# eriksandstroem/Loopy-SLAM

Hardware: AMD Instinct MI355X
Metric: rays/s (track+map, Replica room0 per-frame budget, 640x480 synthetic RGB-D) (higher is better)
Workload: dtype f32 (decoder products as split products on the 16-bit matrix pipe: fp16x3 forward, bf16x6 / pre-scaled fp16x3 backward, fp32 accumulate; weight gradients on pre-scaled fp16x3 too)

## Files before the change

### loopy_slam_amd/csrc/lk_bwd2.hip

```cpp
#include "lk_common.h"
#include "lk_kernels.h"
#include "lk_adam_dev.h"
#include "lk_exposure_dev.h"

using namespace lkw;

LK_CHAIN_DEFINE(bwd2)

__device__ __forceinline__ void interp_bwd_block(const LkInterpBwdArgs& a, int block) {
    const int sub = (int)threadIdx.x & 7;
    const int p_raw = block * 32 + ((int)threadIdx.x >> 3);
    const bool live = p_raw < a.P;
    const int pidx = live ? p_raw : a.P - 1;
    const bool has = a.nbr_count[pidx] >= a.min_nn;
    const bool color = (a.flags & LK_FLAG_STAGE_COLOR) != 0;
    const bool relpos = (a.flags & LK_FLAG_REL_POS) != 0;
    const bool do_col = color && !relpos;
    int id[LK_K];
    float w[LK_K];
    {
        const int4 i0 = *reinterpret_cast<const int4*>(a.nbr_idx + (size_t)pidx * LK_K);
        const int4 i1 = *reinterpret_cast<const int4*>(a.nbr_idx + (size_t)pidx * LK_K + 4);
        const float4 w0 = *reinterpret_cast<const float4*>(a.nbr_w + (size_t)pidx * LK_K);
        const float4 w1 = *reinterpret_cast<const float4*>(a.nbr_w + (size_t)pidx * LK_K + 4);
        id[0] = i0.x; id[1] = i0.y; id[2] = i0.z; id[3] = i0.w; id[4] = i1.x; id[5] = i1.y; id[6] = i1.z; id[7] = i1.w;
        w[0] = w0.x; w[1] = w0.y; w[2] = w0.z; w[3] = w0.w; w[4] = w1.x; w[5] = w1.y; w[6] = w1.z; w[7] = w1.w;
    }
    const float4 dcg = *reinterpret_cast<const float4*>(a.dc_geo + (size_t)pidx * LK_C + sub * 4);
    float4 dcc = make_float4(0.f, 0.f, 0.f, 0.f);
    if (do_col) dcc = *reinterpret_cast<const float4*>(a.dc_col + (size_t)pidx * LK_C + sub * 4);
    if (!(a.flags & LK_FLAG_GRAD_RAYS)) return;
    float dwn[LK_K];
#pragma unroll
    for (int j = 0; j < LK_K; ++j) {
        float part = 0.0f;
        if (has && w[j] != 0.0f) {
            const float4 g = lk_feat4(a.geo_feats, (a.flags & LK_FLAG_FEATS_F16) != 0, (size_t)id[j] * LK_C + sub * 4);
            part = dcg.x * g.x + dcg.y * g.y + dcg.z * g.z + dcg.w * g.w;
            if (do_col) {
                const float4 c = lk_feat4(a.col_feats, (a.flags & LK_FLAG_FEATS_F16) != 0, (size_t)id[j] * LK_C + sub * 4);
                part += dcc.x * c.x + dcc.y * c.y + dcc.z * c.z + dcc.w * c.w;
            }
        }
        part = lk_sum8<true>(part);
        if (color && relpos && a.dw_rel && has) part += a.dw_rel[(size_t)pidx * LK_K + j];
        dwn[j] = part;
    }
    LK_STAMPW(7);
    const int r = pidx / a.S;
    const float z = a.z[pidx];
    const float px = lk_madd_rn(a.rays_o[3 * r], a.rays_d[3 * r], z);
    const float py = lk_madd_rn(a.rays_o[3 * r + 1], a.rays_d[3 * r + 1], z);
    const float pz = lk_madd_rn(a.rays_o[3 * r + 2], a.rays_d[3 * r + 2], z);
    const float r2 = a.r2_ray ? a.r2_ray[r] : a.r2_static;
    float dpx = 0.0f, dpy = 0.0f, dpz = 0.0f;
    if (has) {
        float wr[LK_K], ex[LK_K], ey[LK_K], ez[LK_K];
        float S = 0.0f, dot = 0.0f;
#pragma unroll
        for (int j = 0; j < LK_K; ++j) {
            wr[j] = 0.0f; ex[j] = ey[j] = ez[j] = 0.0f;
            if (id[j] >= 0) {
                const float x = a.pos[3 * (size_t)id[j]], y = a.pos[3 * (size_t)id[j] + 1], zz = a.pos[3 * (size_t)id[j] + 2];
                const float D = lk_dist2(px, py, pz, x, y, zz);
                if (D <= r2) { wr[j] = 1.0f / (D + 1e-10f); ex[j] = x - px; ey[j] = y - py; ez[j] = zz - pz; }
            }
            S += wr[j];
            dot += dwn[j] * w[j];
        }
        const float invS = 1.0f / fmaxf(S, 1e-12f);
#pragma unroll
        for (int j = 0; j < LK_K; ++j) {
            if (wr[j] != 0.0f) {
                const float dw = (dwn[j] - dot) * invS;
                const float dD = -wr[j] * wr[j] * dw;
                dpx += dD * (-2.0f) * ex[j]; dpy += dD * (-2.0f) * ey[j]; dpz += dD * (-2.0f) * ez[j];
            }
        }
    }
    if (live && sub == 0) {
        if (a.dp_embed) { const float4 e = *reinterpret_cast<const float4*>(a.dp_embed + (size_t)pidx * 4); dpx += e.x; dpy += e.y; dpz += e.z; }
        if (color && a.dp_embed_col) { const float4 e = *reinterpret_cast<const float4*>(a.dp_embed_col + (size_t)pidx * 4); dpx += e.x; dpy += e.y; dpz += e.z; }
        if (color && relpos && a.dp_rel) { const float4 e = *reinterpret_cast<const float4*>(a.dp_rel + (size_t)pidx * 4); dpx += e.x; dpy += e.y; dpz += e.z; }
        *reinterpret_cast<float4*>(a.dp_total + (size_t)pidx * 4) = make_float4(dpx, dpy, dpz, 0.0f);
    }
    LK_STAMPW(8);
    if (a.pose_part) {
        __shared__ float s_pp[4][12];
        float v[12];
        const bool mine = live && sub == 0;
        const float d0 = mine ? (a.pix_i[r] - a.cx) / a.fx : 0.0f, d1 = mine ? -(a.pix_j[r] - a.cy) / a.fy : 0.0f, d2 = mine ? -1.0f : 0.0f;
        const float gx = mine ? dpx : 0.0f, gy = mine ? dpy : 0.0f, gz = mine ? dpz : 0.0f;
        const float zx = gx * z, zy = gy * z, zz = gz * z;
        v[0] = zx * d0; v[1] = zx * d1; v[2] = zx * d2; v[3] = zy * d0; v[4] = zy * d1; v[5] = zy * d2; v[6] = zz * d0; v[7] = zz * d1; v[8] = zz * d2;
        v[9] = gx; v[10] = gy; v[11] = gz;
#pragma unroll
        for (int q = 0; q < 12; ++q) {
#pragma unroll
            for (int o = 32; o >= 8; o >>= 1) v[q] += __shfl_xor(v[q], o);
        }
        const int wv = (int)threadIdx.x >> 6;
        if (lk_lane() == 0) {
#pragma unroll
            for (int q = 0; q < 12; ++q) s_pp[wv][q] = v[q];
        }
        __syncthreads();
        if (threadIdx.x < 12) a.pose_part[(size_t)block * 12 + threadIdx.x] = (s_pp[0][threadIdx.x] + s_pp[1][threadIdx.x]) + (s_pp[2][threadIdx.x] + s_pp[3][threadIdx.x]);
    }
    LK_STAMPW(9);
}
__global__ __launch_bounds__(256) void k_interp_bwd(LkInterpBwdArgs a) { interp_bwd_block(a, (int)blockIdx.x); }
__global__ __launch_bounds__(256) void k_interp_bwd_x(LkInterpBwdArgs a, ExposureStepArgs xa, const float* __restrict__ part, int n_part) {
    if (blockIdx.x + 1 == gridDim.x) { lk_exposure_step_body(xa, part, n_part); return; }
    interp_bwd_block(a, (int)blockIdx.x);
}

__global__ __launch_bounds__(256) void k_seg_count(LkFeatScatterArgs a) {
    const long long row = (long long)blockIdx.x * 256 + (int)threadIdx.x;
    if (row >= (long long)a.P * LK_K) return;
    const int y = (int)blockIdx.y;
    const long long grow = (long long)y * a.P * LK_K + row;
    const int s = (int)(row >> 3);
    const int idx = a.nbr_idx[grow];
    int rk = -1;
    const bool skipped = a.live_rays && s >= a.live_rays[y] * a.S;
    if (!skipped && idx >= 0 && a.nbr_w[grow] != 0.0f && a.nbr_count[(size_t)y * a.P + s] >= a.min_nn && (!a.row_mask || a.row_mask[idx])) {
        const int key = a.key_of ? a.key_of[idx] : idx;
        if (key >= 0) rk = atomicAdd(a.seg_cnt + (size_t)y * a.cnt_stride + key, 1);
    }
    a.seg_rank[grow] = rk;
}
__global__ __launch_bounds__(256) void k_seg_place(LkFeatScatterArgs a) {
    const long long row = (long long)blockIdx.x * 256 + (int)threadIdx.x;
    if (row >= (long long)a.P * LK_K) return;
    const int y = (int)blockIdx.y;
    const long long base = (long long)y * a.P * LK_K;
    const int32_t* __restrict__ off = a.seg_off + (size_t)y * a.cnt_stride;
    const int rk = a.seg_rank[base + row];
    if (rk >= 0) {
        const int idx = a.nbr_idx[base + row];
        a.seg_list[base + off[a.key_of ? a.key_of[idx] : idx] + rk] = (int)row;
    }
    if (row == 0 && a.seg_total) a.seg_total[y] = off[a.N];
}

__global__ __launch_bounds__(256) void k_seg_rank_det(LkFeatScatterArgs a) {
    const long long row = (long long)blockIdx.x * 256 + (int)threadIdx.x;
    if (row >= (long long)a.P * LK_K) return;
    const int y = (int)blockIdx.y;
    const long long base = (long long)y * a.P * LK_K;
    if (a.seg_rank[base + row] < 0) return;
    const int32_t* __restrict__ off = a.seg_off + (size_t)y * a.cnt_stride;
    const int idx = a.nbr_idx[base + row];
    const int key = a.key_of ? a.key_of[idx] : idx;
    int rk = 0;
    for (int i = off[key], e = off[key + 1]; i < e; ++i) rk += a.seg_list[base + i] < (int)row;
    a.seg_rank[base + row] = rk;
}

#define LK_DW2_LDS_SAMPLES 32
__device__ __forceinline__ void dw2_body(const float* __restrict__ dc, const float* __restrict__ w_sum, const float* __restrict__ hbar,
                                         int P_all, const int32_t* __restrict__ live_rays, int S, float* __restrict__ part, int bx, int nb) {
    const int P = live_rays ? min(P_all, *live_rays * S) : P_all;
    __shared__ __attribute__((aligned(16))) float s_h[LK_DW2_LDS_SAMPLES][128];
    __shared__ float s_a[LK_DW2_LDS_SAMPLES][33];
    const int t = (int)threadIdx.x, n = t >> 3, k0 = 16 * (t & 7);
    float acc[16], bsum = 0.0f;
#pragma unroll
    for (int i = 0; i < 16; ++i) acc[i] = 0.0f;
    for (int s0 = bx * 64; s0 < P; s0 += nb * 64) {
        for (int half = 0; half < 64; half += LK_DW2_LDS_SAMPLES) {
            const int ns = min(LK_DW2_LDS_SAMPLES, P - s0 - half);
            if (ns <= 0) break;
            __syncthreads();
#pragma unroll
            for (int q = 0; q < LK_DW2_LDS_SAMPLES * 32 / 256; ++q) {
                const int e = q * 256 + t, sm = e >> 5;
                float4 v = make_float4(0.f, 0.f, 0.f, 0.f);
                float av = 0.0f;
                if (sm < ns) {
                    v = reinterpret_cast<const float4*>(hbar + (size_t)(s0 + half + sm) * 128)[e & 31];
                    av = w_sum[s0 + half + sm] * dc[(size_t)(s0 + half + sm) * LK_C + (e & 31)];
                }
                reinterpret_cast<float4*>(&s_h[sm][0])[e & 31] = v;
                s_a[sm][e & 31] = av;
            }
            __syncthreads();
#pragma unroll 4
            for (int sm = 0; sm < LK_DW2_LDS_SAMPLES; ++sm) {
                const float av = s_a[sm][n];
                const float4* __restrict__ hb = reinterpret_cast<const float4*>(&s_h[sm][k0]);
                bsum += av;
#pragma unroll
                for (int q = 0; q < 4; ++q) {
                    const float4 v = hb[q];
                    acc[4 * q] = fmaf(av, v.x, acc[4 * q]); acc[4 * q + 1] = fmaf(av, v.y, acc[4 * q + 1]);
                    acc[4 * q + 2] = fmaf(av, v.z, acc[4 * q + 2]); acc[4 * q + 3] = fmaf(av, v.w, acc[4 * q + 3]);
                }
            }
        }
    }
    float* __restrict__ out = part + (size_t)bx * (32 * 129) + n * 129;
#pragma unroll
    for (int i = 0; i < 16; ++i) out[k0 + i] = acc[i];
    if (k0 == 0) out[128] = bsum;
}
#define LK_GATHER_CHUNK 16
__device__ __forceinline__ void col_reduce_body(const float* __restrict__ part, int n_parts, int width, float* __restrict__ out, int bx, float (*sh)[32],
                                                const LkStepRider& sr);
__global__ __launch_bounds__(256) void k_feat_gather(LkFeatScatterArgs a) {
    const int xb = a.x_on ? 1 : 0;
    if (xb && blockIdx.x == 0) { lk_exposure_step_body(a.x, nullptr, 0); return; }
    if ((int)blockIdx.x - xb < a.dw2_blocks) {
        dw2_body(a.dw2_dc, a.dw2_w_sum, a.dw2_hbar, a.P, a.dw2_live, a.dw2_S, a.dw2_part, (int)blockIdx.x - xb, a.dw2_blocks);
        return;
    }
    const int bx = (int)blockIdx.x - xb - a.dw2_blocks;
    if (a.red_part && bx >= a.red_block0) {
        __shared__ float sh[8][32];
        LkStepRider none; none.n_span = 0;
        col_reduce_body(a.red_part, a.red_n, a.red_width, a.red_out, bx - a.red_block0, sh, none);
        return;
    }
    const int c = (int)threadIdx.x & 31;
    long long i0 = ((long long)bx * 8 + ((int)threadIdx.x >> 5)) * LK_GATHER_CHUNK;
    const int total = a.seg_total ? *a.seg_total : a.seg_off[a.N];
    if (i0 >= total) return;
    const long long e = min(i0 + LK_GATHER_CHUNK, (long long)total);
    if (i0 > 0) {
        const int prev = a.nbr_idx[a.seg_list[i0 - 1]];
        while (i0 < e && a.nbr_idx[a.seg_list[i0]] == prev) ++i0;
        if (i0 == e) return;
    }
    const bool col = a.dfeat != nullptr || a.dc_col != nullptr;
    int cur = -1;
    float sg = 0.0f, sc = 0.0f;
    for (long long b = i0; b < total; b += 4) {
        int row[4], idx[4];
        float vg[4], vc[4];
#pragma unroll
        for (int u = 0; u < 4; ++u) row[u] = a.seg_list[min(b + u, (long long)total - 1)];
#pragma unroll
        for (int u = 0; u < 4; ++u) {
            idx[u] = a.nbr_idx[row[u]];
            const float w = a.nbr_w[row[u]];
            const int s = row[u] >> 3;
            vg[u] = w * a.dc_geo[(size_t)s * LK_C + c];
            vc[u] = a.dfeat ? a.dfeat[(size_t)row[u] * LK_C + c] : (a.dc_col ? w * a.dc_col[(size_t)s * LK_C + c] : 0.0f);
        }
        bool done = false;
#pragma unroll
        for (int u = 0; u < 4; ++u) {
            if (done || b + u >= total) { done = true; continue; }
            if (idx[u] != cur) {
                if (b + u >= e) { done = true; continue; }
                if (cur >= 0) {
                    atomicAdd(a.g_geo_feats + (size_t)cur * LK_C + c, sg);
                    if (col) atomicAdd(a.g_col_feats + (size_t)cur * LK_C + c, sc);
                    if (a.act_flag && c == 0) a.act_flag[cur] = 1;
                }
                cur = idx[u]; sg = 0.0f; sc = 0.0f;
            }
            sg += vg[u]; sc += vc[u];
        }
        if (done) break;
    }
    atomicAdd(a.g_geo_feats + (size_t)cur * LK_C + c, sg);
    if (col) atomicAdd(a.g_col_feats + (size_t)cur * LK_C + c, sc);
    if (a.act_flag && c == 0) a.act_flag[cur] = 1;
}

__global__ __launch_bounds__(256) void k_rays_bwd(LkRaysBwdArgs a) {
    const int r = blockIdx.x * 256 + (int)threadIdx.x;
    if (r >= a.R) return;
    float ox = 0.f, oy = 0.f, oz = 0.f, dx = 0.f, dy = 0.f, dz = 0.f;
    for (int s = 0; s < a.S; ++s) {
        const int p = r * a.S + s;
        const float4 g = *reinterpret_cast<const float4*>(a.dp_total + (size_t)p * 4);
        const float z = a.z[p];
        ox += g.x; oy += g.y; oz += g.z;
        dx = fmaf(g.x, z, dx); dy = fmaf(g.y, z, dy); dz = fmaf(g.z, z, dz);
    }
    a.g_rays_o[3 * r] = ox; a.g_rays_o[3 * r + 1] = oy; a.g_rays_o[3 * r + 2] = oz;
    a.g_rays_d[3 * r] = dx; a.g_rays_d[3 * r + 1] = dy; a.g_rays_d[3 * r + 2] = dz;
}

__device__ __forceinline__ float rp_embed_unit(const float* __restrict__ B, int u, float a0, float a1, float a2) {
    const int xi = (u < 10) ? u : u - 10;
    const float x = lk_fourier_arg(a0, a1, a2, B[xi], B[10 + xi], B[20 + xi]);
    return (u < 10) ? lk_sinf(x) : lk_cosf(x);
}

template <bool F16, bool H16 = false>
__device__ __forceinline__ void relpos_bwd_wave(const LkRelposBwdArgs& a, int sample0, float* __restrict__ part) {
    typedef BwdPiece<H16> PC;
    typedef typename PC::T Piece;
    constexpr float SC = H16 ? 1024.0f : 1.0f, ISC = H16 ? 1.0f / 1024.0f : 1.0f;
    const int lane = lk_lane();
    const int h = lane >> 5;
    const int j = lane & 31;
    const int sample = sample0 + (j >> 3);
    const bool live = sample < a.P;
    const int sp = live ? sample : a.P - 1;
    const int nb_i = j & 7;
    const int r = sp / a.S;
    const float z = a.z[sp];
    const float px = lk_madd_rn(a.rays_o[3 * r], a.rays_d[3 * r], z);
    const float py = lk_madd_rn(a.rays_o[3 * r + 1], a.rays_d[3 * r + 1], z);
    const float pz = lk_madd_rn(a.rays_o[3 * r + 2], a.rays_d[3 * r + 2], z);
    int idx = a.nbr_idx[(size_t)sp * LK_K + nb_i];
    const bool has = a.nbr_count[sp] >= a.min_nn;
    float wgt = (idx >= 0 && has && live) ? a.nbr_w[(size_t)sp * LK_K + nb_i] : 0.0f;
    if (idx < 0) idx = 0;
    const float a0 = __fmul_rn(LK_TWO_PI, __fsub_rn(a.pos[3 * (size_t)idx], px));
    const float a1 = __fmul_rn(LK_TWO_PI, __fsub_rn(a.pos[3 * (size_t)idx + 1], py));
    const float a2 = __fmul_rn(LK_TWO_PI, __fsub_rn(a.pos[3 * (size_t)idx + 2], pz));
    const float* __restrict__ W = a.W;
    const u32x4* __restrict__ FB = reinterpret_cast<const u32x4*>(a.Wfrag);
    const u32x4* __restrict__ FP = FB + (H16 ? FRAGB_U4 : 0);
    const size_t frow = (size_t)idx * LK_C;
    constexpr bool f16 = F16;
    const bool want_w = !H16 && (a.flags & LK_FLAG_GRAD_WEIGHTS) != 0;
    const bool want_p = (a.flags & LK_FLAG_GRAD_RAYS) != 0;
    f32x16 x0, x1;
#pragma unroll
    for (int g = 0; g < 4; ++g) {
        const int u0 = 8 * g + 4 * h;
        if (u0 < ER) {
#pragma unroll
            for (int t = 0; t < 4; ++t) x0[4 * g + t] = rp_embed_unit(W + R_EB, u0 + t, a0, a1, a2);
        } else {
            const float4 v = lk_feat4(a.col_feats, f16, frow + (u0 - ER));
            x0[4 * g] = v.x; x0[4 * g + 1] = v.y; x0[4 * g + 2] = v.z; x0[4 * g + 3] = v.w;
        }
    }
    x1 = lk_zero16();
#pragma unroll
    for (int g = 0; g < 3; ++g) {
        const int u0 = 32 + 8 * g + 4 * h;
        if (u0 < KR) {
            const float4 v = lk_feat4(a.col_feats, f16, frow + (u0 - ER));
            x1[4 * g] = v.x; x1[4 * g + 1] = v.y; x1[4 * g + 2] = v.z; x1[4 * g + 3] = v.w;
        }
    }
    LK_STAMPW(1);
    f32x16 hid[4];
#pragma unroll
    for (int nb = 0; nb < 4; ++nb) hid[nb] = lk_rowvec_tile(W + R_B1, nb * 32, lane);
    const u32x4* __restrict__ FH = FB + FRAGB_U4;
    lk_gemm_h3<4, 2>(hid, FH + FM20_FWDH, 4, 0, 0, x0, 0, lane);
    lk_gemm_h3<4, 2>(hid, FH + FM20_FWDH, 4, 2, 0, x1, 0, lane);
#pragma unroll
    for (int nb = 0; nb < 4; ++nb) {
#pragma unroll
        for (int q = 0; q < 16; ++q) hid[nb][q] = lk_softplus100(hid[nb][q]);
    }
    LK_STAMP(2);
    f32x16 dout[1];
    const float* dcrow = a.dc_col + (size_t)sp * LK_C;
#pragma unroll
    for (int g = 0; g < 4; ++g) {
        const float4 v = *reinterpret_cast<const float4*>(dcrow + 8 * g + 4 * h);
        dout[0][4 * g] = v.x; dout[0][4 * g + 1] = v.y; dout[0][4 * g + 2] = v.z; dout[0][4 * g + 3] = v.w;
    }
    if (want_p) {
        f32x16 out[1];
        out[0] = lk_rowvec_tile(W + R_B2, 0, lane);
#pragma unroll
        for (int kb = 0; kb < 4; ++kb) lk_gemm_h3<1, 2>(out, FH + FM21_FWDH, 1, 2 * kb, 0, hid[kb], 0, lane);
        float part = 0.0f;
#pragma unroll
        for (int q = 0; q < 16; ++q) part = fmaf(dout[0][q], out[0][q], part);
        part += __shfl_xor(part, 32);
        if (live && h == 0) a.dw_rel[(size_t)sp * LK_K + nb_i] = (has && a.nbr_idx[(size_t)sp * LK_K + nb_i] >= 0) ? part : 0.0f;
    }
    {
        const float ws = H16 ? wgt * SC : wgt;
#pragma unroll
        for (int q = 0; q < 16; ++q) dout[0][q] *= ws;
    }
    if (want_w) {
        float wsum = wgt;
        wsum = lk_sum8<true>(wsum);
        if (live && h == 0 && nb_i == 0) a.w_sum[sp] = wsum;
    }
    f32x16 (&dhid)[4] = hid;
    const Piece db0 = PC::split(dout[0], 0), db1 = PC::split(dout[0], 1);
    Piece fa0 = PC::load(FP + PC::tr(21), 4, 0, 0, lane), fa1 = PC::load(FP + PC::tr(21), 4, 1, 0, lane);
    Piece fx[4];
#pragma unroll
    for (int nb = 0; nb < 4; ++nb) {
        f32x16 t = lk_zero16();
        t = PC::mma(fa0, db0, t);
        t = PC::mma(fa1, db1, t);
        if (nb < 3) {
            fa0 = PC::load(FP + PC::tr(21), 4, 0, nb + 1, lane);
            fa1 = PC::load(FP + PC::tr(21), 4, 1, nb + 1, lane);
        } else {
#pragma unroll
            for (int q = 0; q < 4; ++q) fx[q] = PC::load(FP + PC::tr(20), 2, q >> 1, q & 1, lane);
        }
        __builtin_amdgcn_sched_barrier(0);
        if (want_w) {
#pragma unroll
            for (int g = 0; g < 4; ++g) {
                float v[4];
#pragma unroll
                for (int tt = 0; tt < 4; ++tt) {
                    float sred = wgt * hid[nb][4 * g + tt];
                    sred = lk_sum8<true>(sred);
                    v[tt] = sred;
                }
                if (live && nb_i == 0)
                    *reinterpret_cast<float4*>(a.hbar + (size_t)sp * 128 + nb * 32 + 8 * g + 4 * h) = make_float4(v[0], v[1], v[2], v[3]);
            }
        }
#pragma unroll
        for (int q = 0; q < 16; ++q) dhid[nb][q] = t[q] * lk_softplus100_grad_from_out(hid[nb][q]);
    }
    LK_STAMP(3);
    f32x16 dx[2];
    dx[0] = lk_zero16(); dx[1] = lk_zero16();
#pragma unroll
    for (int nb = 0; nb < 4; ++nb) {
#pragma unroll
        for (int G = 0; G < 2; ++G) {
            const Piece b = PC::split(dhid[nb], G);
#pragma unroll
            for (int kb = 0; kb < 2; ++kb)
                dx[kb] = PC::mma(nb == 0 ? fx[2 * G + kb] : PC::load(FP + PC::tr(20), 2, 2 * nb + G, kb, lane), b, dx[kb]);
        }
    }
    if (H16) {
#pragma unroll
        for (int kb = 0; kb < 2; ++kb)
#pragma unroll
            for (int q = 0; q < 16; ++q) dx[kb][q] *= ISC;
    }
    __builtin_amdgcn_sched_barrier(0);
    LK_STAMP(4);
    if (want_w) {
        if (live) {
            if (h == 0) a.w_eff[(size_t)sp * 8 + nb_i] = wgt;
            float* row = a.rows + ((size_t)sp * 8 + nb_i) * 192;
#pragma unroll
            for (int nb = 0; nb < 4; ++nb)
#pragma unroll
                for (int g = 0; g < 4; ++g)
                    *reinterpret_cast<float4*>(row + nb * 32 + 8 * g + 4 * h) =
                        make_float4(dhid[nb][4 * g], dhid[nb][4 * g + 1], dhid[nb][4 * g + 2], dhid[nb][4 * g + 3]);
#pragma unroll
            for (int g = 0; g < 4; ++g) {
                *reinterpret_cast<float4*>(row + 128 + 8 * g + 4 * h) = make_float4(x0[4 * g], x0[4 * g + 1], x0[4 * g + 2], x0[4 * g + 3]);
                *reinterpret_cast<float4*>(row + 160 + 8 * g + 4 * h) = make_float4(x1[4 * g], x1[4 * g + 1], x1[4 * g + 2], x1[4 * g + 3]);
            }
        }
    }
    float dax = 0.0f, day = 0.0f, daz = 0.0f;
    const float* B = W + R_EB;
    float fder[12];
    {
        const float r0 = __shfl_xor(h ? x0[4] : x0[8], 32), r1 = __shfl_xor(h ? x0[5] : x0[9], 32);
        const float r2 = __shfl_xor(x0[2], 32), r3 = __shfl_xor(x0[3], 32);
        fder[0] = x0[6]; fder[1] = x0[7]; fder[2] = r0; fder[3] = r1;
        fder[4] = h ? -r2 : x0[10]; fder[5] = h ? -r3 : x0[11]; fder[6] = -x0[0]; fder[7] = -x0[1];
        fder[8] = -r2; fder[9] = -r3; fder[10] = -x0[4]; fder[11] = -x0[5];
    }
#pragma unroll
    for (int tile = 0; tile < 2; ++tile)
#pragma unroll
        for (int g = 0; g < 4; ++g) {
            const int u0 = 32 * tile + 8 * g + 4 * h;
            const bool is_emb = u0 < ER;
            if (tile == 0 && g < 3) {
#pragma unroll
                for (int t = 0; t < 4; ++t) {
                    const int u = u0 + t;
                    const int xi = is_emb ? ((u < 10) ? u : u - 10) : 0;
                    const float b0 = B[xi], b1 = B[10 + xi], b2 = B[20 + xi];
                    float gx = 0.0f;
                    if (is_emb) gx = dx[tile][4 * g + t] * fder[4 * g + t];
                    if (want_p) {
                        dax = fmaf(gx * LK_TWO_PI, b0, dax); day = fmaf(gx * LK_TWO_PI, b1, day); daz = fmaf(gx * LK_TWO_PI, b2, daz);
                    }
                    if (want_w) {
                        const float s0 = lk_half_wave_sum(gx * a0), s1 = lk_half_wave_sum(gx * a1), s2 = lk_half_wave_sum(gx * a2);
                        if ((lane & 31) == LK_HWS_LANE && is_emb) {
                            atomicAdd(part + xi, s0);
                            atomicAdd(part + 10 + xi, s1);
                            atomicAdd(part + 20 + xi, s2);
                        }
                    }
                }
            }
            if (!is_emb && u0 < KR) {
                if ((a.flags & LK_FLAG_GRAD_FEATS) && live)
                    *reinterpret_cast<float4*>(a.dfeat + ((size_t)sp * 8 + nb_i) * LK_C + (u0 - ER)) =
                        make_float4(dx[tile][4 * g], dx[tile][4 * g + 1], dx[tile][4 * g + 2], dx[tile][4 * g + 3]);
            }
        }
    if (want_p) {
        dax += __shfl_xor(dax, 32); day += __shfl_xor(day, 32); daz += __shfl_xor(daz, 32);
        dax = lk_sum8<true>(dax);
        day = lk_sum8<true>(day);
        daz = lk_sum8<true>(daz);
        if (live && h == 0 && nb_i == 0) *reinterpret_cast<float4*>(a.dp_rel + (size_t)sp * 4) = make_float4(-dax, -day, -daz, 0.0f);
    }
}

template <bool F16>
__global__ __launch_bounds__(256, 2) void k_relpos_bwd(LkRelposBwdArgs a) {
    __shared__ float s_part[4][32];
    const bool want_w = (a.flags & LK_FLAG_GRAD_WEIGHTS) != 0;
    const int w = (int)threadIdx.x >> 6;
    if (want_w) {
        if (threadIdx.x < 128) (&s_part[0][0])[threadIdx.x] = 0.0f;
        __syncthreads();
    }
    const int sample0 = (blockIdx.x * 4 + w) * 4;
    if (sample0 < a.P) relpos_bwd_wave<F16>(a, sample0, s_part[w]);
    if (want_w) {
        __syncthreads();
        if (threadIdx.x < 32)
            a.part_br[(size_t)blockIdx.x * 32 + threadIdx.x] = s_part[0][threadIdx.x] + s_part[1][threadIdx.x] +
                                                                 s_part[2][threadIdx.x] + s_part[3][threadIdx.x];
    }
}

template <bool F16, bool H16>
__global__ __launch_bounds__(512) void k_relpos_interp_bwd(LkRelposBwdArgs rb, LkInterpBwdArgs ib) {
    __shared__ float s_dummy[32];
    const int w = (int)threadIdx.x >> 6;
    const int sample0 = (int)blockIdx.x * 32 + 4 * w;
    LK_STAMP(0);
    if (sample0 < rb.P) relpos_bwd_wave<F16, H16>(rb, sample0, s_dummy);
    LK_STAMP(5);
    __syncthreads();
    LK_STAMP(6);
    if (w >= 4) return;
    interp_bwd_block(ib, (int)blockIdx.x);
}

#define RPF_XU 56
#define RPF_DU 64
#define RPF_STAGE_HALVES ((2 * RPF_XU + 2 * RPF_DU) * 32)
#define RPF_SC 1024.0f
#define RPF_ISC (1.0f / 1024.0f)

struct RpfLane {
    int wr[2];
    int rd_j[2];
    int rd_x[2];
};
__device__ __forceinline__ RpfLane rpf_lane(int lane) {
    const int h = lane >> 5, row = lane & 31;
    RpfLane L;
#pragma unroll
    for (int k = 0; k < 2; ++k) L.wr[k] = 4 * h * 32 + ((((row >> 3) ^ (2 * k + h)) & 3) << 3) + (row & 7);
    const int xu = (32 + row < RPF_XU) ? 32 + row : RPF_XU - 1;
#pragma unroll
    for (int kk = 0; kk < 2; ++kk) {
        L.rd_j[kk] = row * 32 + ((((2 * kk + h) ^ (row >> 2)) & 3) << 3);
        L.rd_x[kk] = xu * 32 + ((((2 * kk + h) ^ (xu >> 2)) & 3) << 3);
    }
    return L;
}
__device__ __forceinline__ void rpf_stage(uint16_t* __restrict__ hi, uint16_t* __restrict__ lo, const LkH8& b, int G, int unit0,
                                          int n_units, const RpfLane& L, int h) {
#pragma unroll
    for (int j = 0; j < 4; ++j) {
        const int c = unit0 + 2 * (j & 1) + 8 * (2 * G + (j >> 1));
        if (c + 4 < n_units || (c < n_units && h == 0)) {
// ... 788 lines not shown
```

Measured before the change: 19.10 million.

## Tile segment ranking through LDS and warp-cooperatively scan segments in feature gather

k_seg_rank_det now walks the sorted segment list per block, stages the shared range of candidate rows in LDS and counts smaller rows with vectorized int4 reads, instead of each thread rescanning its segment in global memory. k_feat_gather now has 32 lanes load 32 list entries at a time and find segment heads with shuffles and ballots, then broadcasts rows so each lane accumulates its feature channel. The aim is to cut redundant serial global loads and the per-thread boundary search. In exchange the code is more complex and relies on 32-lane sub-warp shuffle and ballot semantics on 64-wide wavefronts.

```diff
diff --git a/loopy_slam_amd/csrc/lk_bwd2.hip b/loopy_slam_amd/csrc/lk_bwd2.hip
--- a/loopy_slam_amd/csrc/lk_bwd2.hip
+++ b/loopy_slam_amd/csrc/lk_bwd2.hip
@@ -145,17 +145,42 @@
 }
 
 __global__ __launch_bounds__(256) void k_seg_rank_det(LkFeatScatterArgs a) {
-    const long long row = (long long)blockIdx.x * 256 + (int)threadIdx.x;
-    if (row >= (long long)a.P * LK_K) return;
-    const int y = (int)blockIdx.y;
+    __shared__ __attribute__((aligned(16))) int s_row[256];
+    __shared__ int s_span[2];
+    const int y = (int)blockIdx.y, t = (int)threadIdx.x;
     const long long base = (long long)y * a.P * LK_K;
-    if (a.seg_rank[base + row] < 0) return;
     const int32_t* __restrict__ off = a.seg_off + (size_t)y * a.cnt_stride;
-    const int idx = a.nbr_idx[base + row];
-    const int key = a.key_of ? a.key_of[idx] : idx;
+    const int32_t* __restrict__ list = a.seg_list + base;
+    const int total = off[a.N];
+    const int p0 = (int)blockIdx.x * 256;
+    if (p0 >= total) return;
+    const int p = p0 + t, last = min(p0 + 256, total) - 1;
+    int row = 0, lo = 0, hi = 0;
+    if (p <= last) {
+        row = list[p];
+        const int idx = a.nbr_idx[base + row];
+        const int key = a.key_of ? a.key_of[idx] : idx;
+        lo = off[key]; hi = off[key + 1];
+    }
+    if (t == 0) s_span[0] = lo;
+    if (p == last) s_span[1] = hi;
+    __syncthreads();
+    const int A = s_span[0], B = s_span[1];
     int rk = 0;
-    for (int i = off[key], e = off[key + 1]; i < e; ++i) rk += a.seg_list[base + i] < (int)row;
-    a.seg_rank[base + row] = rk;
+    for (int t0 = A; t0 < B; t0 += 256) {
+        if (t0 + t < B) s_row[t] = list[t0 + t];
+        __syncthreads();
+        const int j0 = max(lo, t0) - t0, j1 = min(hi, t0 + 256) - t0;
+        int j = j0;
+        for (; j < j1 && (j & 3); ++j) rk += s_row[j] < row;
+        for (; j + 4 <= j1; j += 4) {
+            const int4 v = *reinterpret_cast<const int4*>(&s_row[j]);
+            rk += (v.x < row) + (v.y < row) + (v.z < row) + (v.w < row);
+        }
+        for (; j < j1; ++j) rk += s_row[j] < row;
+        __syncthreads();
+    }
+    if (p <= last) a.seg_rank[base + row] = rk;
 }
 
 #define LK_DW2_LDS_SAMPLES 32
@@ -206,6 +231,7 @@
     if (k0 == 0) out[128] = bsum;
 }
 #define LK_GATHER_CHUNK 16
+static_assert(LK_GATHER_CHUNK < 32, "k_feat_gather: a chunk lies inside the first 32-entry window");
 __device__ __forceinline__ void col_reduce_body(const float* __restrict__ part, int n_parts, int width, float* __restrict__ out, int bx, float (*sh)[32],
                                                 const LkStepRider& sr);
 __global__ __launch_bounds__(256) void k_feat_gather(LkFeatScatterArgs a) {
@@ -222,52 +248,73 @@
         col_reduce_body(a.red_part, a.red_n, a.red_width, a.red_out, bx - a.red_block0, sh, none);
         return;
     }
-    const int c = (int)threadIdx.x & 31;
-    long long i0 = ((long long)bx * 8 + ((int)threadIdx.x >> 5)) * LK_GATHER_CHUNK;
+    const int c = (int)threadIdx.x & 31, hsh = (int)threadIdx.x & 32;
+    const long long i0 = ((long long)bx * 8 + ((int)threadIdx.x >> 5)) * LK_GATHER_CHUNK;
     const int total = a.seg_total ? *a.seg_total : a.seg_off[a.N];
     if (i0 >= total) return;
-    const long long e = min(i0 + LK_GATHER_CHUNK, (long long)total);
-    if (i0 > 0) {
-        const int prev = a.nbr_idx[a.seg_list[i0 - 1]];
-        while (i0 < e && a.nbr_idx[a.seg_list[i0]] == prev) ++i0;
-        if (i0 == e) return;
-    }
+    const int* __restrict__ list = a.seg_list;
     const bool col = a.dfeat != nullptr || a.dc_col != nullptr;
-    int cur = -1;
+    int prev = i0 > 0 ? a.nbr_idx[list[i0 - 1]] : -1;
+    int cur = -1, lo = -1;
     float sg = 0.0f, sc = 0.0f;
-    for (long long b = i0; b < total; b += 4) {
-        int row[4], idx[4];
-        float vg[4], vc[4];
-#pragma unroll
-        for (int u = 0; u < 4; ++u) row[u] = a.seg_list[min(b + u, (long long)total - 1)];
-#pragma unroll
-        for (int u = 0; u < 4; ++u) {
-            idx[u] = a.nbr_idx[row[u]];
-            const float w = a.nbr_w[row[u]];
-            const int s = row[u] >> 3;
-            vg[u] = w * a.dc_geo[(size_t)s * LK_C + c];
-            vc[u] = a.dfeat ? a.dfeat[(size_t)row[u] * LK_C + c] : (a.dc_col ? w * a.dc_col[(size_t)s * LK_C + c] : 0.0f);
-        }
-        bool done = false;
-#pragma unroll
-        for (int u = 0; u < 4; ++u) {
-            if (done || b + u >= total) { done = true; continue; }
-            if (idx[u] != cur) {
-                if (b + u >= e) { done = true; continue; }
-                if (cur >= 0) {
-                    atomicAdd(a.g_geo_feats + (size_t)cur * LK_C + c, sg);
-                    if (col) atomicAdd(a.g_col_feats + (size_t)cur * LK_C + c, sc);
-                    if (a.act_flag && c == 0) a.act_flag[cur] = 1;
+    bool live = true;
+    for (long long b = i0;; b += 32) {
+        const bool in = live && b + c < total;
+        const int row = in ? list[b + c] : 0;
+        const int idx = in ? a.nbr_idx[row] : -1;
+        const float w = in ? a.nbr_w[row] : 0.0f;
+        int before = __shfl_up(idx, 1, 32);
+        if (c == 0) before = prev;
+        prev = __shfl(idx, 31, 32);
+        const unsigned head = (unsigned)(__ballot(in && idx != before) >> hsh);
+        const int n = __popc((unsigned)(__ballot(in) >> hsh));
+        const int ce = (int)max(i0 + LK_GATHER_CHUNK - b, 0ll);
+        const unsigned in_chunk = (1u << ce) - 1u;
+        if (lo < 0) {
+            const unsigned own = head & in_chunk;
+            lo = own ? __builtin_ctz(own) : 32;
+        } else lo = 0;
+        const unsigned stop = head & ~in_chunk;
+        const int hi = min(stop ? __builtin_ctz(stop) : 32, n);
+#pragma unroll 1
+        for (int g = 0; g < 32; g += 16) {
+            if (!__any(lo < g + 16 && hi > g)) continue;
+            float vg[16], vc[16];
+#pragma unroll
+            for (int u = 0; u < 16; ++u) {
+                const int ru = __shfl(row, g + u, 32);
+                const float wu = __shfl(w, g + u, 32);
+                vg[u] = 0.0f; vc[u] = 0.0f;
+                if (g + u >= lo && g + u < hi) {
+                    const int s = ru >> 3;
+                    vg[u] = wu * a.dc_geo[(size_t)s * LK_C + c];
+                    if (col) vc[u] = a.dfeat ? a.dfeat[(size_t)ru * LK_C + c] : wu * a.dc_col[(size_t)s * LK_C + c];
                 }
-                cur = idx[u]; sg = 0.0f; sc = 0.0f;
-            }
-            sg += vg[u]; sc += vc[u];
-        }
-        if (done) break;
-    }
-    atomicAdd(a.g_geo_feats + (size_t)cur * LK_C + c, sg);
-    if (col) atomicAdd(a.g_col_feats + (size_t)cur * LK_C + c, sc);
-    if (a.act_flag && c == 0) a.act_flag[cur] = 1;
+            }
+#pragma unroll
+            for (int u = 0; u < 16; ++u) {
+                const int iu = __shfl(idx, g + u, 32);
+                if (g + u >= lo && g + u < hi) {
+                    if ((head >> (g + u)) & 1u) {
+                        if (cur >= 0) {
+                            atomicAdd(a.g_geo_feats + (size_t)cur * LK_C + c, sg);
+                            if (col) atomicAdd(a.g_col_feats + (size_t)cur * LK_C + c, sc);
+                            if (a.act_flag && c == 0) a.act_flag[cur] = 1;
+                        }
+                        cur = iu; sg = 0.0f; sc = 0.0f;
+                    }
+                    sg += vg[u]; sc += vc[u];
+                }
+            }
+        }
+        live = live && lo < 32 && stop == 0 && n == 32;
+        if (!__any(live)) break;
+    }
+    if (cur >= 0) {
+        atomicAdd(a.g_geo_feats + (size_t)cur * LK_C + c, sg);
+        if (col) atomicAdd(a.g_col_feats + (size_t)cur * LK_C + c, sc);
+        if (a.act_flag && c == 0) a.act_flag[cur] = 1;
+    }
 }
 
 __global__ __launch_bounds__(256) void k_rays_bwd(LkRaysBwdArgs a) {
```

Measured after the change: 19.37 million, median of 6. +1.4%, better.
